# oksuman/FHE-Sorting

Measured on AMD Instinct MI355X. Metric: encrypted sort seconds + ciphertext-mults/sec, N=1024 @ ringDim 2^16, higher is better.
Workload: dtype u64; 1 GPU; DirectSort N=1024, ringDim 2^16, depth 39, scale 2^40, 161 rotation keys, CompositeSign(3, 5, 2), dnum 3, OpenFHE PS split; N=1024, ring_dim=65536, mult_depth=39, scale_bits=40, ps_split=openfhe, special_primes=10, lanes_per_gpu=2, max_stack=32, parallelism=batch-shard x1, collective=none

## Files before the change

### fhe-sorting_amd/csrc/algo/fhesort.cpp

```cpp
#include "fhesort.hpp"

#include <algorithm>
#include <chrono>
#include <cstdio>
#include <cstdlib>
#include <cmath>
#include <fstream>
#include <map>
#include <mutex>
#include <optional>
#include <stdexcept>
#include <tuple>
#include <exception>
#include <thread>

namespace fhe {

namespace {

int ceil_log2(long x) {
    int r = 0;
    while ((1L << r) < x) ++r;
    return r;
}
void trim_zeros(std::vector<double> &a) {
    while (a.size() > 1 && a.back() == 0.0) a.pop_back();
}
size_t ps_chunk() {
    static const size_t v = [] {
        const char *e = std::getenv("FHE_PS_CHUNK");
        const int c = e ? std::atoi(e) : 32;
        return (size_t)std::min(32, std::max(1, c));
    }();
    return v;
}
bool fold_scalars() {
    static const bool v = [] {
        const char *e = std::getenv("FHE_MUL_FOLD_SCALARS");
        return e ? std::atoi(e) != 0 : true;
    }();
    return v;
}

int openfhe_ps_depth(int d) {
    if (d < 5) return ceil_log2(d) + 1;
    static const int band_top[] = {5, 13, 27, 59, 119, 247, 495, 1007, 2031, 2204};
    for (int i = 0; i < 10; ++i)
        if (d <= band_top[i]) return 3 + i;
    const double f = std::floor(std::log2(std::sqrt(d / 2.0)));
    long best = -1;
    int depth = 0;
    for (long k = 1; k <= d; ++k) {
        if (std::fabs(std::floor(std::log2((double)k)) - f) > 1) continue;
// ... 107 lines not shown
                chunk.push_back(i);
        std::vector<int> idx;
        for (size_t c : chunk)
            for (size_t i = 1; i < leaves[c].a.size(); ++i)
                if (leaves[c].a[i] != 0.0) idx.push_back((int)i);
        std::sort(idx.begin(), idx.end());
        idx.erase(std::unique(idx.begin(), idx.end()), idx.end());
        std::vector<const Ciphertext *> xs;
        for (int i : idx) xs.push_back(T.at(i).get());
        std::vector<std::vector<double>> rows;
        for (size_t c : chunk) {
            std::vector<double> row;
            for (int i : idx) row.push_back((size_t)i < leaves[c].a.size() ? leaves[c].a[i] : 0.0);
            rows.push_back(row);
        }
        auto outs = cc.linear_sums_to(xs, rows, target, !raw);
        for (size_t g = 0; g < chunk.size(); ++g) {
            CtPtr r = std::move(outs[g]);
            if (!raw && leaves[chunk[g]].a[0] != 0.0) cc.add_const_inplace(r, leaves[chunk[g]].a[0]);
            ready[chunk[g]] = r;
        }
    }
    CtPtr leaf() {
        const size_t i = next_leaf++;
        const Leaf &L = leaves.at(i);
        if (!has_terms(L.a)) {
            CtPtr r = cc.trivial_const(0.0, L.target, T[1]->slots, T[1]->batch);
            if (L.a[0] != 0.0) cc.add_const_inplace(r, L.a[0]);
            return r;
        }
        if (!ready.count(i)) evaluate_chunk(i);
        CtPtr r = ready.at(i);
        ready.erase(i);
        return r;
// ... 284 lines not shown
        for (size_t c : chunk)
            for (int i = 1; i <= k; ++i)
                if (P->leaves[c].a[i] != 0.0) idx.push_back(i);
        std::sort(idx.begin(), idx.end());
        idx.erase(std::unique(idx.begin(), idx.end()), idx.end());
        const int target = lk + L0.mm - 1 + (L0.raw ? 1 : 0);
        if (idx.empty()) throw std::logic_error("openfhe split: leaf without T terms");
        std::vector<const Ciphertext *> xs;
        for (int i : idx) xs.push_back(T[i].get());
        std::vector<std::vector<double>> rows;
        for (size_t c : chunk) {
            std::vector<double> row;
            for (int i : idx) row.push_back(P->leaves[c].a[i]);
            rows.push_back(row);
        }
        auto outs = cc.linear_sums_to(xs, rows, target, !L0.raw);
        for (size_t g = 0; g < chunk.size(); ++g) {
            CtPtr r = std::move(outs[g]);
            if (!L0.raw && P->leaves[chunk[g]].a[0] != 0.0) cc.add_const_inplace(r, P->leaves[chunk[g]].a[0]);
            ready[chunk[g]] = r;
        }
    }
    CtPtr leaf(int i) {
        if (!ready.count(i)) evaluate_chunk(i);
        CtPtr r = ready.at(i);
        ready.erase(i);
        return r;
    }
    CtPtr node(const OFNode &N) {
        CtPtr cu = N.cu >= 0 ? leaf(N.cu) : nullptr;
        const CtPtr &a = T2[N.mm - 1];
        const double c0 = cu ? 0.0 : N.c0;
        CtPtr qu = N.qn ? node(*N.qn) : leaf(N.qleaf);
        if (N.sn) {
// ... 1791 lines not shown
```

### fhe-sorting_amd/csrc/device/kernels.hip

```cpp
#include <fcntl.h>
#include <signal.h>
#include <sys/syscall.h>
#include <ucontext.h>
#include <unistd.h>

#include <atomic>
#include <cstdlib>
#include <mutex>
#include "kernels.hpp"

#include <cstdlib>
#include <stdexcept>
#include <utility>
#include <type_traits>
#include <string>

namespace fhe {
namespace dev {

namespace {

constexpr int NT = 256;
inline int conv_chunk(int logN, int targets, int zdim) {
    static const int force = [] {
// ... 422 lines not shown
    for (int i = 0; i < A.m; ++i) {
        const ulonglong2 x = ld2(A.x[i] + xo);
        mac128(r0, x.x, w[i]);
        mac128(r1, x.y, w[i]);
    }
    st2(out + off + k, make_ulonglong2(reduce128(r0, md), reduce128(r1, md)));
}
constexpr int MLS_G = 10, MLS_M = 32;
struct MultiLinArgs {
    u64 *out[MLS_G];
    const u64 *x[MLS_M];
    size_t xseg[MLS_M];
    int64_t K[MLS_G * MLS_M];
    uint8_t sh[MLS_G * MLS_M];
    int m, G, accumulate;
};
template <int G>
__global__ __launch_bounds__(NT) void k_linear_sum_multi(MultiLinArgs A, size_t seg, const Mod *mods, int logN) {
    __shared__ Split30 w[G * MLS_M];
    const size_t n = (size_t)1 << logN;
    const int l = blockIdx.y;
    const Mod md = mods[l];
    for (int t = threadIdx.x; t < G * MLS_M; t += NT) w[t] = split30((t % MLS_M) < A.m ? smod(A.K[t], A.sh[t], md) : 0);
    __syncthreads();
    const size_t k = (size_t)blockIdx.x * NT + threadIdx.x;
    if (k >= n) return;
    const size_t ln = (size_t)l * n + k, oo = (size_t)blockIdx.z * seg + ln;
    Acc128 run[G];
#pragma unroll
    for (int g = 0; g < G; ++g) run[g].lo = A.accumulate ? A.out[g][oo] : 0;
    for (int base = 0; base < A.m; base += 16) {
        const int end = min(A.m, base + 16);
        Acc4 s[G];
        u64 xv[16];
#pragma unroll
        for (int u = 0; u < 16; ++u) xv[u] = base + u < end ? A.x[base + u][(size_t)blockIdx.z * A.xseg[base + u] + ln] : 0;
#pragma unroll
        for (int u = 0; u < 16; ++u) {
            if (base + u < end) {
                const Split30 x = split30(xv[u]);
#pragma unroll
                for (int g = 0; g < G; ++g) mac4(s[g], x, w[g * MLS_M + base + u]);
            }
        }
#pragma unroll
// ... 97 lines not shown

__device__ __forceinline__ v4i bytes_hilo(u64 y0, u64 y1) {
    return v4i{(int)(uint32_t)(y0 >> 32), (int)(uint32_t)(y1 >> 32), (int)(uint32_t)y0, (int)(uint32_t)y1};
}
typedef int v16i __attribute__((ext_vector_type(16)));

constexpr int LS_CH_MAX = 4096;
struct LeafArgs {
    u64 *out[LEAF_G];
    const u64 *x[LEAF_M];
    uint32_t xseg[LEAF_M];
    const int64_t *K;
    const uint8_t *sh;
    int m, G, accumulate;
    int six;
};
#ifndef FHE_LF_NC
#define FHE_LF_NC 2
#endif
constexpr int LF_NC = FHE_LF_NC, LF_NT = 256;
#ifndef FHE_LF_WPE
#define FHE_LF_WPE 3
#endif
template <int KS, int NG>
__global__ __launch_bounds__(LF_NT) __attribute__((amdgpu_waves_per_eu(FHE_LF_WPE, 8))) void k_leaf_sums_mfma(LeafArgs A, size_t seg, const Mod *mods, int logN,
                                                          int chunk) {
    __shared__ u64 etab[4 * NG][8 * KS];
    __shared__ u64 corr[4 * NG];
    __shared__ const u64 *xptr[8 * KS];
    __shared__ size_t xoff[8 * KS];
    __shared__ u64 *optr[4 * NG];
// ... 6 lines not shown
        const int t = p / (8 * KS), i = p % (8 * KS);
        const u64 c = (t < A.G && i < A.m) ? smod(A.K[t * A.m + i], A.sh[t * A.m + i], md) : 0;
        etab[t][i] = __builtin_bswap64(balanced_digits(c));
    }
    if (tid < 8 * KS) {
        const int i = tid < A.m ? tid : 0;
        xptr[tid] = A.x[i];
        xoff[tid] = (size_t)blockIdx.z * A.xseg[i] + (size_t)l * n;
    }
    __syncthreads();
    if (tid < 4 * ngr) {
        optr[tid] = tid < A.G ? A.out[tid] : nullptr;
        u64 s = 0;
        if (tid < A.G)
            for (int i = 0; i < A.m; ++i) s = add_mod(s, smod(A.K[tid * A.m + i], A.sh[tid * A.m + i], md), md.q);
        corr[tid] = sums_constant(s, md);
    }
    __syncthreads();
    const int lane = tid & 63, wave = tid >> 6, col = lane & 15, lg = lane >> 4;
    const int ta = (lane & 15) >> 2, rr = lane & 3;
    const uint32_t ab = 3 - rr;
    const u64 w1s = shoup_one(md);
    const size_t oo_l = (size_t)blockIdx.z * seg + (size_t)l * n;
    for (size_t nb = (size_t)blockIdx.x * chunk + wave * 16 * LF_NC; nb < (size_t)(blockIdx.x + 1) * chunk && nb < n;
         nb += LF_NT / 4 * LF_NC) {
        v4i bf[LF_NC][KS];
#pragma unroll
        for (int ks = 0; ks < KS; ++ks) {
            const int i0 = 8 * ks + 2 * lg;
            const gu64 *p0 = to_global(xptr[i0]) + xoff[i0] + nb + col;
            const gu64 *p1 = to_global(xptr[i0 + 1]) + xoff[i0 + 1] + nb + col;
// ... 182 lines not shown
                img[2 * (((grp * 2 + (b >> 2)) * KS + ks) * 64 + lane) + half] = e;
            }
        }
    }
    if (tid < 8 * KS) {
        const int i = tid < A.m ? tid : 0;
        xptr[tid] = A.x[i];
        xoff[tid] = (size_t)blockIdx.z * A.xseg[i] + (size_t)l * n;
    }
    __syncthreads();
    if (tid < 4 * ngr) {
        optr[tid] = tid < A.G ? A.out[tid] : nullptr;
        u64 s = 0;
        for (int i = 0; i < A.m; ++i) s = add_mod(s, psum[tid][i], md.q);
        const u64 b126 = mul_shoup(reduce64(1ull << 62, md), md.r64, md.r64s, md.q);
        corr[tid] = sub_mod(mul_barrett(s, 128, md), b126, md.q);
        cfp[tid] = mul_barrett(s, 128, md);
    }
    __syncthreads();
    const int lane = tid & 63, wave = tid >> 6, col = lane & 15, lg = lane >> 4;
    const u64 w1s = shoup_one(md);
    const double qd = (double)md.q, qid = 1.0 / qd;
    const size_t oo_l = (size_t)blockIdx.z * seg + (size_t)l * n;
    for (size_t nb = (size_t)blockIdx.x * chunk + wave * 16 * LFF_NC; nb < (size_t)(blockIdx.x + 1) * chunk && nb < n;
         nb += LFF_NT / 4 * LFF_NC) {
        v4i bf[LFF_NC][KS];
#pragma unroll
        for (int ks = 0; ks < KS; ++ks) {
            const int i0 = 8 * ks + 2 * lg;
            const gu64 *p0 = to_global(xptr[i0]) + xoff[i0] + nb + col;
            const gu64 *p1 = to_global(xptr[i0 + 1]) + xoff[i0 + 1] + nb + col;
#pragma unroll
// ... 1804 lines not shown
        launch_clocked("k_linear_sum", B, k_linear_sum, ew_grid(logN, limbs, segs), dim3(NT), st, out, A, seg, mods,
                       logN);
        if (m == 0) break;
    }
}
int leaf_fold_enabled() {
    static const int v = [] {
        const char *e = std::getenv("FHE_LEAF_FOLD");
        return e ? std::atoi(e) : 1;
    }();
    return v;
}
bool linear_sums_on_mfma(int logN) { return use_mfma_sums(MF_LIN) && logN >= 8; }
void ew_linear_sum_multi(u64 *const *outs, int G, const u64 *const *xs, const size_t *xseg, const int64_t *K, int m,
                         int limbs, int segs, size_t seg, const Mod *mods, int logN, hipStream_t st,
                         const uint8_t *sh, const int64_t *dK, const uint8_t *dsh) {
    if (limbs <= 0 || segs <= 0 || G <= 0 || m <= 0) return;
    if (G > LEAF_G) throw std::invalid_argument("ew_linear_sum_multi: at most LEAF_G outputs per call");
    const size_t n = (size_t)1 << logN;
    if (linear_sums_on_mfma(logN) && dK && dsh && m <= LEAF_M) {
        {
            LeafArgs A{};
            A.m = m;
            A.G = G;
            A.accumulate = 0;
            for (int g = 0; g < G; ++g) A.out[g] = outs[g];
            A.six = leaf_six_enabled_host();
            for (int i = 0; i < A.m; ++i) {
                A.x[i] = xs[i];
                A.xseg[i] = (uint32_t)xseg[i];
            }
            A.K = dK;
            A.sh = dsh;
            const double B = 8.0 * (A.m + (double)G * (1 + A.accumulate)) * limbs * segs * (double)n;
            size_t ch = std::min<size_t>(LS_CH_MAX, n);
            while (ch > 256 && (n / ch) * (size_t)limbs * (size_t)segs < 2048) ch /= 2;
            const dim3 grid((unsigned)((n + ch - 1) / ch), (unsigned)limbs, (unsigned)segs);
            const int ngc = (G + 3) / 4 <= 1 ? 1 : (G + 3) / 4 <= 2 ? 2 : (G + 3) / 4 <= 4 ? 3 : 4;
            if (leaf_fold_enabled() && n >= 2 * (size_t)LFF_NT) {
                size_t chf = std::min<size_t>(LS_CH_MAX, n);
                while (chf > 2 * (size_t)LFF_NT && (n / chf) * (size_t)limbs * (size_t)segs < 1024) chf /= 2;
                const dim3 gridf((unsigned)((n + chf - 1) / chf), (unsigned)limbs, (unsigned)segs);
                dispatch_int<1, 8>((A.m + 7) / 8, [&](auto ks) {
                    dispatch_int<1, 4>(ngc, [&](auto ng) {
                        constexpr int KS = decltype(ks)::value, NG = 1 << (decltype(ng)::value - 1);
                        launch_clocked(inst_name<KS, NG>("k_leaf_sums_fold"), B, k_leaf_sums_fold<KS, NG>, gridf,
                                       dim3(LFF_NT), st, A, seg, mods, logN, (int)chf);
                    });
// ... 5 lines not shown
                    constexpr int KS = decltype(ks)::value, NG = 1 << (decltype(ng)::value - 1);
                    launch_clocked(inst_name<KS, NG>("k_leaf_sums_mfma"), B, k_leaf_sums_mfma<KS, NG>, grid, dim3(LF_NT),
                                   st, A, seg, mods, logN, (int)ch);
                });
            });
        }
        return;
    }
    for (int g0 = 0; g0 < G; g0 += MLS_G) {
        const int Gp = std::min(MLS_G, G - g0);
        for (int base = 0; base < m; base += MLS_M) {
            MultiLinArgs A{};
            A.m = std::min(MLS_M, m - base);
            A.G = Gp;
            A.accumulate = base > 0;
            for (int g = 0; g < Gp; ++g) A.out[g] = outs[g0 + g];
            for (int i = 0; i < A.m; ++i) {
                A.x[i] = xs[base + i];
                A.xseg[i] = xseg[base + i];
                for (int g = 0; g < Gp; ++g) {
                    A.K[g * MLS_M + i] = K[(size_t)(g0 + g) * m + base + i];
                    A.sh[g * MLS_M + i] = sh ? sh[(size_t)(g0 + g) * m + base + i] : 0;
                }
            }
            const double B = 8.0 * (A.m + (double)Gp * (1 + A.accumulate)) * limbs * segs * (double)n;
            const dim3 grid = pt_grid(logN, limbs, segs);
            switch (Gp) {
#define MLS_CASE(g)                                                                                               \
    case g:                                                                                                       \
        launch_clocked(inst_name<g>("k_linear_sum_multi"), B, k_linear_sum_multi<g>, grid, dim3(NT), st, A, seg, mods, \
// ... 723 lines not shown
```

### fhe-sorting_amd/csrc/device/kernels.hpp

```cpp
#pragma once
#include <string>
#include <utility>
#include <vector>
#include <hip/hip_runtime.h>
#include <hip/hip_ext.h>
#include <cstddef>
#include <cstdint>

#include "modmath.hpp"

namespace fhe {
namespace dev {

struct NttTables {
    const ulonglong2 *fwd2;
    const ulonglong2 *inv2;
    const u64 *ninv, *ninv_s;
    const Mod *mods;
    int logN;
    const double *fwdd = nullptr, *invd = nullptr;
    const double2 *qd = nullptr;
    const uint8_t *fp_host = nullptr;
};
bool ntt_fp_prime(u64 q);
// ... 54 lines not shown
    size_t seg_d = 0;
    const u64 *c1 = nullptr, *c1s = nullptr;
    const u64 *c2 = nullptr, *c2s = nullptr;
    const u64 *src = nullptr;
    size_t seg_src = 0;
    int64_t scalar = 0;
    int scalar_sh = 0;
    bool raw = false;
    int lsegb = 0, segs = 0;
    int zs0 = 0, zn0 = 1 << 30, zs1 = 0;
    __host__ __device__ int limb_of(int z) const { return z < zn0 ? zs0 + z : zs1 + (z - zn0); }
    const u64 *d2 = nullptr;
    size_t seg_d2 = 0;
    const u64 *key = nullptr;
    int nall = 0;
};
void ntt_inverse_from(u64 *dst, const u64 *src, size_t seg_src, int limbs, int segs, size_t seg, const int *pmap,
                      const NttTables &T, hipStream_t st, bool raw = false);
void ntt_forward_rescale(u64 *tmp, int limbs, int segs, const NttFuse &F, const NttTables &T, hipStream_t st);
void ntt_forward_multail(u64 *corr, int limbs, int segs, const NttFuse &F, const NttTables &T, hipStream_t st);
void ntt_forward_multail_own(u64 *corr, int limbs, int segs, const NttFuse &F, const NttTables &T, hipStream_t st);
void ntt_forward_ksfinish(u64 *conv, int limbs, int segs, const NttFuse &F, const NttTables &T, hipStream_t st);
void ntt_row_pass(u64 *data, int limbs, int segs, size_t seg, const int *pmap, const NttTables &T, hipStream_t st,
                  bool forward);
void ntt_forward_mapped(u64 *data, int count, int segs, size_t seg, const int *smap, const int *pmap,
                        const NttTables &T, hipStream_t st);

struct Seg {
    size_t o, a, b;
};
// ... 22 lines not shown
                   const u64 *const *xs, const int64_t *K, const uint8_t *sh, int m, size_t xseg, const Mod *mods,
                   int logN, hipStream_t st, const u64 *a2 = nullptr, size_t sa2 = 0, int64_t aK = 0, int ash = 0,
                   int64_t oK = 0, int osh = 0);
void ew_sum_members(u64 *out, const u64 *in, int members, int limbs, const Mod *mods, int logN, hipStream_t st);
int tensor_cols_per_thread();
void ew_tensor_cols(u64 *d01, u64 *d2, const u64 *a, const u64 *const *cols, int P, int limbs, int members, size_t sa,
                    const Mod *mods, int logN, hipStream_t st);
void ew_sum_member_groups(u64 *out, const u64 *in, int groups, int per_group, int limbs, bool accumulate,
                          const Mod *mods, int logN, hipStream_t st);
void ew_linear_sum(u64 *out, const u64 *const *xs, const int64_t *K, int m, int limbs, int segs, size_t seg,
                   size_t xseg, const Mod *mods, int logN, hipStream_t st, bool accumulate = false,
                   const uint8_t *sh = nullptr);
constexpr int LEAF_G = 32, LEAF_M = 64;
void ew_linear_sum_multi(u64 *const *outs, int G, const u64 *const *xs, const size_t *xseg, const int64_t *K, int m,
                         int limbs, int segs, size_t seg, const Mod *mods, int logN, hipStream_t st,
                         const uint8_t *sh, const int64_t *dK, const uint8_t *dsh);
bool linear_sums_on_mfma(int logN);
void ew_mul_plain_sum(u64 *out, const u64 *const *cts, const u64 *const *pts, int m, int limbs, int members,
                      size_t cmember, size_t cpoly, const Mod *mods, int logN, hipStream_t st);
int plain_sum_tile();
double plain_sum_batches_limb_units(int m, int nb, int tile);
void ew_mul_plain_sum_batches(u64 *out, const u64 *const *cts, const u64 *const *pts, int m, int nb, int limbs,
                              size_t cpoly, const Mod *mods, int logN, hipStream_t st);
int plain_sum_groups_tile();
void ew_mul_plain_sum_groups(u64 *out, const u64 *in, const u64 *const *pts, int m, int groups, int limbs,
                             const Mod *mods, int logN, hipStream_t st);
int sub_add_plain_tile();
void ew_sub_add_plain_stacked(u64 *out, const u64 *a, const u64 *const *bs, const u64 *const *ps, int members,
                              int limbs, const Mod *mods, int logN, hipStream_t st);
int sub_pm_const_tile();
void ew_sub_pm_const_stacked(u64 *out, const u64 *a, const u64 *const *bs, int members, int64_t K, int sh, int limbs,
// ... 106 lines not shown
```

### fhe-sorting_amd/csrc/device/ntt.hip

```cpp
#include <hip/hip_ext.h>

#include <cstdlib>
#include <map>
#include <atomic>
#include <mutex>
#include <stdexcept>
#include <string>
#include <type_traits>
#include <utility>
#include <vector>

#include "kernels.hpp"

namespace fhe {
namespace dev {

namespace {

constexpr int NTB = 256;

template <int Lo, int Hi, typename F>
void dispatch_int(int v, F &&f) {
    if constexpr (Lo > Hi) {
        throw std::invalid_argument("unsupported digit count " + std::to_string(v));
// ... 348 lines not shown
template <bool FWD>
__device__ __forceinline__ int row_final_index(int t, int r) {
    constexpr RowLayout L = row_layout<FWD>(FWD ? 8 : 7);
    return lane_index(L, t) + reg_index(L, r);
}
int &row_shfl_enabled() {
    static int v = [] {
        const char *e = std::getenv("FHE_NTT_ROW_SHFL");
        return e ? std::atoi(e) : 15;
    }();
    return v;
}

enum { NTT_PLAIN = 0, NTT_LIFT = 1, NTT_RESCALE = 2, NTT_MULTAIL = 3, NTT_KSFINISH = 4, NTT_MULTAIL_OWN = 5 };

template <int PB, int EB, bool COLS, int MODE, bool SH, bool FULL, bool TWL = false, bool FP = false>
__device__ __forceinline__ void ntt_fwd_body(u64 *data, size_t seg, const int *pmap, const int *smap, int logN,
                                             const NttTables &Tb, const NttFuse &F) {
    static_assert(!SH || (!COLS && PB == 8 && EB == 4), "shuffle row pass: 16 lanes x 16 coefficients");
    constexpr int E = 1 << EB;
    constexpr int RB = PB - EB;
    constexpr int T = 1 << RB;
    constexpr int NB = nthreads<PB, COLS>() / T;
    constexpr int G = E >> RB;
    constexpr int LEN = 1 << PB;
    constexpr bool SPLIT = COLS && G >= 2;
    constexpr int TPB = SPLIT ? PB - (EB - RB) : PB;
    constexpr bool X32 = lds32<COLS>() && !SPLIT;
    __shared__ u64 tile[SH ? 1 : X32 ? (lds_words<TPB, NB, COLS>() + 1) / 2 : lds_words<TPB, NB, COLS>()];
    uint32_t *const t32 = reinterpret_cast<uint32_t *>(tile);
    constexpr bool CTW = FHE_NTT_COL_TWL && COLS && !SPLIT && PB == 8 && nthreads<PB, COLS>() == 256;
    using TW = TwT<FP>;
    __shared__ TW twc[CTW ? 256 : 1];

    const size_t n = (size_t)1 << logN;
    const int k2 = COLS ? logN - PB : 0;
    const int limb = F.limb_of(blockIdx.z);
    const int p = pmap ? __builtin_amdgcn_readfirstlane(pmap[limb]) : limb;
    int t, tr;
    if (COLS) {
        tr = threadIdx.x % NB;
        t = NB == 64 ? __builtin_amdgcn_readfirstlane(threadIdx.x / NB) : threadIdx.x / NB;
    } else {
        tr = threadIdx.x / T;
        t = threadIdx.x % T;
    }
    const int zseg = SH ? (int)blockIdx.x * (1 << F.lsegb) + (tr & ((1 << F.lsegb) - 1)) : (int)blockIdx.x;
    const size_t tid_global = SH ? (size_t)blockIdx.y * (NB >> F.lsegb) + (tr >> F.lsegb)
                                 : (size_t)blockIdx.y * NB + tr;
    const bool valid = FULL || (tid_global < ((size_t)1 << (logN - PB)) && (!SH || zseg < F.segs));
    u64 *a = data + (size_t)zseg * seg + (smap ? (size_t)__builtin_amdgcn_readfirstlane(smap[limb]) : (size_t)limb) * n;
    const u64 q = Tb.mods[p].q, q2 = 2 * q, q4 = 4 * q, nq = (u64)0 - q;
    const TW *tw;
    if constexpr (FP) tw = Tb.fwdd + (size_t)p * n;
    else tw = Tb.fwd2 + (size_t)p * n;
    Ar A{q4, nq, 0.0, 0.0};
    if constexpr (FP) {
        const double2 qd = Tb.qd[p];
        A.q = qd.x;
        A.qi = qd.y;
    }
    const double fin = FP ? FP_TWO52 + (COLS ? FP_FWD_COL_IN : FP_FWD_COL_OUT) * A.q : 0.0;
    constexpr bool CBUF = FHE_NTT_COL_BUF && COLS && FULL;
    const int S0 = COLS ? 0 : logN - PB;
    if (CTW) twc[threadIdx.x] = tw[threadIdx.x];

    u64 x[E];
    if (MODE == NTT_LIFT) {
        const Mod ml = Tb.mods[F.lastp];
        const u64 ql = ml.q, qh = ql >> 1;
        const u64 kl = F.scalar ? smod64(F.scalar, F.scalar_sh, ml) : 0;
        const u64 *src = F.last + (size_t)zseg * F.seg_last;
        const auto rs = limb_rsrc(src);
        const int vo = (int)((((size_t)t << k2) + tid_global) * 8);
#pragma unroll
        for (int r = 0; r < E; ++r) {
            const int idx = t + T * r;
            u64 c = CBUF ? bload64(rs, vo, (T * r << k2) * 8)
                         : valid ? src[(size_t)idx * ((size_t)1 << k2) + tid_global] : 0;
            if (F.scalar) c = mul_barrett(c, kl, ml);
            x[r] = c > qh ? q - (ql - c) : c;
        }
    } else if constexpr (CBUF) {
// ... 394 lines not shown
            v = scale ? mul_shoup(x[r], ni, nis, q) : COLS ? (x[r] >= q2 ? x[r] - q2 : x[r]) : x[r];
        }
        if constexpr (CBUF)
            bstore64(rso, vso, (T * r << k2) * 8, v);
        else if (valid)
            a[off] = v;
    }
}

#ifndef FHE_NTT_COL_WPE
#define FHE_NTT_COL_WPE 1
#endif
template <int PB, int EB, bool COLS, int MODE, bool FULL, bool FP>
__global__ __launch_bounds__((nthreads<PB, COLS>())) __attribute__((amdgpu_waves_per_eu(COLS ? FHE_NTT_COL_WPE : 1, 8))) void k_ntt_fwd(
    u64 *data, size_t seg, const int *pmap, const int *smap, int logN, NttTables Tb, NttFuse F) {
    ntt_fwd_body<PB, EB, COLS, MODE, false, FULL, false, FP>(data, seg, pmap, smap, logN, Tb, F);
}
template <int PB, int EB, bool COLS, bool FULL, bool FP>
__global__ __launch_bounds__((nthreads<PB, COLS>())) __attribute__((amdgpu_waves_per_eu(COLS ? FHE_NTT_COL_WPE : 1, 8))) void k_ntt_inv(
    u64 *data, size_t seg, const int *pmap, const int *smap, int logN, NttTables Tb, NttFuse F) {
    ntt_inv_body<PB, EB, COLS, false, FULL, false, FP>(data, seg, pmap, smap, logN, Tb, F);
}
#ifndef FHE_NTT_ROW_WPE
#define FHE_NTT_ROW_WPE 1
#endif
#ifndef FHE_NTT_FP_ROW_WPE
#define FHE_NTT_FP_ROW_WPE 1
#endif
#ifndef FHE_NTT_FP_RESCALE_WPE
#define FHE_NTT_FP_RESCALE_WPE FHE_NTT_FP_ROW_WPE
#endif
template <int MODE, bool FULL, bool TWL, bool FP>
__global__ __launch_bounds__(NTB) __attribute__((amdgpu_waves_per_eu(FP ? (MODE == NTT_RESCALE ? FHE_NTT_FP_RESCALE_WPE : FHE_NTT_FP_ROW_WPE) : TWL ? FHE_NTT_ROW_WPE : 1, 8))) void k_ntt_fwd_row(
    u64 *data, size_t seg, const int *pmap, const int *smap, int logN, NttTables Tb, NttFuse F) {
    ntt_fwd_body<8, 4, false, MODE, true, FULL, TWL, FP>(data, seg, pmap, smap, logN, Tb, F);
}
template <bool FULL, bool TWL, bool FP>
__global__ __launch_bounds__(NTB) __attribute__((amdgpu_waves_per_eu(TWL ? FHE_NTT_ROW_WPE : 1, 8))) void k_ntt_inv_row(
    u64 *data, size_t seg, const int *pmap, const int *smap, int logN, NttTables Tb, NttFuse F) {
    ntt_inv_body<8, 4, false, true, FULL, TWL, FP>(data, seg, pmap, smap, logN, Tb, F);
}
#ifndef FHE_ROW_KS_WPE
#define FHE_ROW_KS_WPE 2
#endif
#ifndef FHE_ROW_KS_WPE1
#define FHE_ROW_KS_WPE1 4
#endif
template <int D, bool FP, bool FULL>
__global__ __launch_bounds__(NTB) __attribute__((amdgpu_waves_per_eu(D == 1 ? FHE_ROW_KS_WPE1 : FHE_ROW_KS_WPE, 8))) void k_ntt_row_ks(u64 *acc, const u64 *ext, const u64 *dntt, const u64 *key,
                                                    int ell, int W, int nall, int alpha, int members,
// ... 154 lines not shown
int &ntt_full_mask() {
    static int v = [] {
        const char *e = std::getenv("FHE_NTT_FULL");
        return e ? std::atoi(e) : 53 | 128;
    }();
    return v;
}
template <bool COLS, bool FWD, int MODE>
constexpr int full_bit() {
    return FWD ? (COLS ? (MODE == NTT_LIFT ? 2 : 1)
                       : MODE == NTT_RESCALE ? 8 : (MODE == NTT_MULTAIL || MODE == NTT_MULTAIL_OWN) ? 16
                       : MODE == NTT_KSFINISH ? 128 : 4)
               : (COLS ? 32 : 64);
}

template <int PB, int EB, bool COLS, bool FWD, int MODE, bool FP>
void launch_pass_one(u64 *data, int limbs, int segs, size_t seg, const int *pmap, const int *smap, const NttTables &T,
                     const NttFuse &F, hipStream_t st) {
    constexpr int NTHR = nthreads<PB, COLS>();
    constexpr int NB = NTHR >> (PB - EB);
    constexpr bool CAN_SH = !COLS && PB == 8 && EB == 4;
    const int mode = row_shfl_enabled();
    const int fwd_bit = (MODE == NTT_MULTAIL || MODE == NTT_MULTAIL_OWN) ? 4 : MODE == NTT_RESCALE ? 8
                        : MODE == NTT_KSFINISH ? 16 : 0;
    const bool sh = CAN_SH && (mode & (FWD ? 2 | fwd_bit : 1)) != 0;
    const int count = 1 << (T.logN - PB);
    dim3 grid((unsigned)segs, (unsigned)((count + NB - 1) / NB), (unsigned)limbs);
    const bool want_full = (ntt_full_mask() & full_bit<COLS, FWD, MODE>()) != 0;
    bool full = want_full && count % NB == 0;
    NttFuse Fs = F;
    if (sh) {
        Fs.lsegb = 0;
        while (Fs.lsegb < 4 && (2 << Fs.lsegb) <= segs) ++Fs.lsegb;
        Fs.segs = segs;
        const int rows_pb = NB >> Fs.lsegb;
        grid = dim3((unsigned)((segs + (1 << Fs.lsegb) - 1) >> Fs.lsegb), (unsigned)((count + rows_pb - 1) / rows_pb),
                    (unsigned)limbs);
        full = want_full && count % rows_pb == 0 && segs % (1 << Fs.lsegb) == 0;
    }
    LaunchClock *clk = launch_clock();
    hipEvent_t e0 = nullptr, e1 = nullptr;
    const int slot = clk ? clk->events(e0, e1) : -1;
    note_launch(FWD ? (COLS ? "k_ntt_fwd(col)" : "k_ntt_fwd(row)") : (COLS ? "k_ntt_inv(col)" : "k_ntt_inv(row)"), grid,
                dim3(NTHR));
    const int rows_blk = 16 >> Fs.lsegb;
    const bool twl = sh && rows_blk <= row_twl_rows() && row_twl_enabled() != 0;
    const unsigned lds_dyn = twl ? (unsigned)(rows_blk * 256 * (FP ? sizeof(double) : sizeof(TwT<false>))) : 0u;
#define FHE_NTT_LAUNCH(K, FF) \
    hipExtLaunchKernelGGL((K), grid, dim3(NTHR), lds_dyn, st, e0, e1, 0, data, seg, pmap, smap, T.logN, T, FF)
    if (FWD && sh) {
        if (full && twl) FHE_NTT_LAUNCH((k_ntt_fwd_row<MODE, true, true, FP>), Fs);
        else if (full) FHE_NTT_LAUNCH((k_ntt_fwd_row<MODE, true, false, FP>), Fs);
        else if (twl) FHE_NTT_LAUNCH((k_ntt_fwd_row<MODE, false, true, FP>), Fs);
        else FHE_NTT_LAUNCH((k_ntt_fwd_row<MODE, false, false, FP>), Fs);
    } else if (FWD) {
        if (full) FHE_NTT_LAUNCH((k_ntt_fwd<PB, EB, COLS, MODE, true, FP>), F);
        else FHE_NTT_LAUNCH((k_ntt_fwd<PB, EB, COLS, MODE, false, FP>), F);
    } else if (sh) {
        if (full && twl) FHE_NTT_LAUNCH((k_ntt_inv_row<true, true, FP>), Fs);
        else if (full) FHE_NTT_LAUNCH((k_ntt_inv_row<true, false, FP>), Fs);
        else if (twl) FHE_NTT_LAUNCH((k_ntt_inv_row<false, true, FP>), Fs);
        else FHE_NTT_LAUNCH((k_ntt_inv_row<false, false, FP>), Fs);
    } else {
        if (full) FHE_NTT_LAUNCH((k_ntt_inv<PB, EB, COLS, true, FP>), F);
        else FHE_NTT_LAUNCH((k_ntt_inv<PB, EB, COLS, false, FP>), F);
    }
#undef FHE_NTT_LAUNCH
    if (clk) {
        const std::string fps = FP ? "true>" : "false>";
        const std::string pe = std::to_string(PB) + ", " + std::to_string(EB) + (COLS ? ", true" : ", false");
        const std::string fl = (full ? "true, " : "false, ") + fps;
        const std::string fl2 = (full ? "true, " : "false, ") + std::string(twl ? "true, " : "false, ") + fps;
        const std::string base = FWD && sh ? "k_ntt_fwd_row<" + std::to_string(MODE) + ", " + fl2
                                 : FWD     ? "k_ntt_fwd<" + pe + ", " + std::to_string(MODE) + ", " + fl
                                 : sh      ? "k_ntt_inv_row<" + fl2
                                           : "k_ntt_inv<" + pe + ", " + fl;
        static std::map<std::string, std::string> names;
        static std::mutex mu;
        const char *ph = launch_phase();
        const std::string key = ph ? base + "@" + ph : base;
        std::lock_guard<std::mutex> lk(mu);
        auto it = names.find(key);
        if (it == names.end()) it = names.emplace(key, key).first;
        const double extra = MODE == NTT_RESCALE ? 1.0 : MODE == NTT_MULTAIL ? 2.0
                             : MODE == NTT_KSFINISH || MODE == NTT_MULTAIL_OWN ? 1.5 : 0.0;
        const double once = MODE == NTT_MULTAIL_OWN ? 2.0 : 0.0;
        clk->record(slot, it->second.c_str(),
                    ((2.0 + extra) * segs + once) * 8.0 * (double)limbs * ((size_t)1 << T.logN));
    }
}

int &ntt_fp_enabled() {
    static int v = [] {
        const char *e = std::getenv("FHE_NTT_FP");
        return e ? std::atoi(e) : 1;
    }();
    return v;
}
struct MapRegistry {
    std::mutex mu;
    std::map<const int *, std::vector<int>> maps;
    std::atomic<unsigned long> gen{0};
};
// ... 339 lines not shown
```

### fhe-sorting_amd/csrc/engine/engine.hip

```cpp
#include <hip/hip_runtime.h>

#include <algorithm>
#include <atomic>
#include <chrono>
#include <cmath>
#include <cstring>
#include <map>
#include <mutex>
#include <set>
#include <stdexcept>
#include <functional>
#include <thread>

#include "../device/kernels.hpp"
#include "engine.hpp"

#define HIP_OK(x)                                                                                     \
    do {                                                                                              \
        hipError_t _e = (x);                                                                          \
        if (_e != hipSuccess)                                                                         \
            throw std::runtime_error(std::string("HIP error ") + hipGetErrorString(_e) + " at " +    \
                                     __FILE__ + ":" + std::to_string(__LINE__));                      \
    } while (0)

// ... 2163 lines not shown
        } else {
            auto sm = I.alloc((size_t)segs * ell * nn * 8);
            u64 *s = static_cast<u64 *>(sm->p);
            dev::ew_linear_sum(s, p.data(), k.data(), (int)p.size(), (int)ell, segs, ell * nn, kv.first * nn, MODS,
                               LOGN, ST, false, sh.data());
            dev::ew_add(t, t, s, (int)ell, segs, seg3(ell * nn, ell * nn, ell * nn), MODS, LOGN, ST);
        }
    }
    ctr.rescale += B;
    auto r = new_ct(target, xs[0]->slots, I.P.delta[target], ell - 1, B);
    I.rescale(t, ell, ell * nn, segs, r->data);
    return r;
}

std::vector<CtPtr> Engine::linear_sums_to(const std::vector<const Ciphertext *> &xs,
                                          const std::vector<std::vector<double>> &c, int target, bool rescale) {
    auto &I = *impl;
    if (target > I.P.L) throw std::runtime_error("linear_sums_to: no levels left");
    if (xs.empty()) throw std::invalid_argument("linear_sums_to: no inputs");
    const int B = xs[0]->batch, segs = 2 * B;
    const size_t nn = n(), ell = I.P.limbs_at(target - 1), m = xs.size();
    const u64 qd = I.P.primes[I.P.L - target + 1];
    count_bytes((2.0 * ell * m + 2.0 * ell) * c.size(), B);
    std::vector<const u64 *> xp(m);
    std::vector<size_t> xseg(m);
    for (size_t i = 0; i < m; ++i) {
        if (xs[i]->level > target - 1) throw std::invalid_argument("linear_sums_to: input level too high");
        if (xs[i]->batch != B) throw std::invalid_argument("linear_sums_to: batch size mismatch");
        xp[i] = xs[i]->data;
        xseg[i] = xs[i]->limbs * nn;
    }
    std::vector<CtPtr> outs;
    const size_t passes = (c.size() + dev::LEAF_G - 1) / dev::LEAF_G, per = (c.size() + passes - 1) / passes;
    const bool mfma = dev::linear_sums_on_mfma(LOGN) && m <= (size_t)dev::LEAF_M;
    for (size_t g0 = 0; g0 < c.size(); g0 += per) {
        const int G = (int)std::min<size_t>(per, c.size() - g0);
        std::vector<int64_t> K((size_t)G * m);
        std::vector<uint8_t> sh((size_t)G * m);
        for (int g = 0; g < G; ++g) {
            if (c[g0 + g].size() != m) throw std::invalid_argument("linear_sums_to: coefficient row size");
            for (size_t i = 0; i < m; ++i) {
                const host::SConst k = host::const_to_target(c[g0 + g][i], I.P.delta[target], qd, xs[i]->scale);
                K[(size_t)g * m + i] = k.k;
                sh[(size_t)g * m + i] = (uint8_t)k.sh;
            }
        }
        auto tm = I.alloc((size_t)G * segs * ell * nn * 8);
        u64 *t = static_cast<u64 *>(tm->p);
        std::vector<u64 *> op(G);
        for (int g = 0; g < G; ++g) op[g] = t + (size_t)g * segs * ell * nn;
        std::pair<const int64_t *, const uint8_t *> dk{nullptr, nullptr};
        if (mfma) dk = I.const_table(K, sh);
        dev::ew_linear_sum_multi(op.data(), G, xp.data(), xseg.data(), K.data(), (int)m, (int)ell, segs, ell * nn,
                                 MODS, LOGN, ST, sh.data(), dk.first, dk.second);
        if (!rescale) {
            for (int g = 0; g < G; ++g) {
                auto r = std::make_shared<Ciphertext>();
                r->mem = tm;
                r->data = op[g];
                r->level = target - 1;
                r->slots = xs[0]->slots;
                r->scale = I.P.delta[target] * (double)qd;
                r->limbs = ell;
                r->batch = B;
                outs.push_back(r);
            }
            ctr.constmult += (u64)G * m * B;
            continue;
        }
// ... 532 lines not shown
```

### fhe-sorting_amd/csrc/engine/engine.hpp

```cpp
#pragma once
#include <array>
#include <complex>
#include <cstddef>
#include <cstdint>
#include <memory>
#include <stdexcept>
#include <string>
#include <vector>

#include "../host/hostmath.hpp"

namespace fhe {

using u64 = uint64_t;
using i64 = int64_t;
using PublicSeed = std::array<uint8_t, 32>;

struct DevMem;

struct Ciphertext {
    std::shared_ptr<DevMem> mem;
    u64 *data = nullptr;
    int level = 0;
    int slots = 0;
// ... 140 lines not shown
    CtPtr rotate_members(const Ciphertext &a, const std::vector<long> &ks);
    CtPtr rotate_sum_hoisted(const Ciphertext &x, const std::vector<long> &ks);
    struct LtGiant {
        long shift = 0;
        std::vector<int> baby;
        std::vector<const Plaintext *> pts;
    };
    CtPtr linear_transform_ext(const Ciphertext &x, const std::vector<long> &baby, const std::vector<LtGiant> &giants);
    std::vector<CtPtr> apply_galois_hoisted(const Ciphertext &a, const std::vector<u64> &gs);
    CtPtr conjugate(const Ciphertext &a);
    CtPtr mod_raise(const Ciphertext &a);
    CtPtr rescale(const Ciphertext &a);
    CtPtr drop_to(const Ciphertext &a, int level);
    CtPtr linear_sum_to(const std::vector<const Ciphertext *> &xs, const std::vector<double> &c, int target);
    std::vector<CtPtr> linear_sums_to(const std::vector<const Ciphertext *> &xs,
                                      const std::vector<std::vector<double>> &c, int target, bool rescale = true);
    CtPtr trivial_const(double c, int level, int slots, int batch = 1);
    CtPtr zero_like(int level, int slots, int batch = 1);
    CtPtr stack(const std::vector<const Ciphertext *> &xs);
    CtPtr member(const Ciphertext &a, int m);
    CtPtr sub_stacked(const Ciphertext &a, const std::vector<const Ciphertext *> &bs);
    CtPtr sub_plain_stacked(const Ciphertext &a, const std::vector<const Plaintext *> &ps);
    CtPtr sub_add_plain_stacked(const Ciphertext &a, const std::vector<const Ciphertext *> &bs,
                                const std::vector<const Plaintext *> &ps);
    CtPtr sub_pm_const_stacked(const Ciphertext &a, const std::vector<const Ciphertext *> &bs, double c);
    CtPtr sum_members(const Ciphertext &a);
    void sum_member_groups(const Ciphertext &a, int groups, CtPtr &acc);
    void reduce_after_allreduce(Ciphertext &ct);

    void ntt_host(u64 *data, int prime_index, int limbs, bool inverse);
    void modup_host(const u64 *d, size_t ell, u64 *ext);
// ... 44 lines not shown
```

Measured before the change: 10990 ciphertext-mults/s.

## Fold leaf constants into linear-sum kernels and loop lifted NTT over limbs

```diff
diff --git a/fhe-sorting_amd/csrc/algo/fhesort.cpp b/fhe-sorting_amd/csrc/algo/fhesort.cpp
--- a/fhe-sorting_amd/csrc/algo/fhesort.cpp
+++ b/fhe-sorting_amd/csrc/algo/fhesort.cpp
@@ -37,6 +37,13 @@
 bool fold_scalars() {
     static const bool v = [] {
         const char *e = std::getenv("FHE_MUL_FOLD_SCALARS");
+        return e ? std::atoi(e) != 0 : true;
+    }();
+    return v;
+}
+bool leaf_const_fold() {
+    static const bool v = [] {
+        const char *e = std::getenv("FHE_LEAF_CONST_FOLD");
         return e ? std::atoi(e) != 0 : true;
     }();
     return v;
@@ -174,10 +181,13 @@
             for (int i : idx) row.push_back((size_t)i < leaves[c].a.size() ? leaves[c].a[i] : 0.0);
             rows.push_back(row);
         }
-        auto outs = cc.linear_sums_to(xs, rows, target, !raw);
+        const bool fold = !raw && leaf_const_fold();
+        std::vector<double> a0;
+        for (size_t c : chunk) a0.push_back(leaves[c].a[0]);
+        auto outs = cc.linear_sums_to(xs, rows, target, !raw, fold ? &a0 : nullptr);
         for (size_t g = 0; g < chunk.size(); ++g) {
             CtPtr r = std::move(outs[g]);
-            if (!raw && leaves[chunk[g]].a[0] != 0.0) cc.add_const_inplace(r, leaves[chunk[g]].a[0]);
+            if (!raw && !fold && a0[g] != 0.0) cc.add_const_inplace(r, a0[g]);
             ready[chunk[g]] = r;
         }
     }
@@ -492,10 +502,13 @@
             for (int i : idx) row.push_back(P->leaves[c].a[i]);
             rows.push_back(row);
         }
-        auto outs = cc.linear_sums_to(xs, rows, target, !L0.raw);
+        const bool fold = !L0.raw && leaf_const_fold();
+        std::vector<double> a0;
+        for (size_t c : chunk) a0.push_back(P->leaves[c].a[0]);
+        auto outs = cc.linear_sums_to(xs, rows, target, !L0.raw, fold ? &a0 : nullptr);
         for (size_t g = 0; g < chunk.size(); ++g) {
             CtPtr r = std::move(outs[g]);
-            if (!L0.raw && P->leaves[chunk[g]].a[0] != 0.0) cc.add_const_inplace(r, P->leaves[chunk[g]].a[0]);
+            if (!L0.raw && !fold && a0[g] != 0.0) cc.add_const_inplace(r, a0[g]);
             ready[chunk[g]] = r;
         }
     }
diff --git a/fhe-sorting_amd/csrc/device/kernels.hip b/fhe-sorting_amd/csrc/device/kernels.hip
--- a/fhe-sorting_amd/csrc/device/kernels.hip
+++ b/fhe-sorting_amd/csrc/device/kernels.hip
@@ -460,21 +460,32 @@
     int64_t K[MLS_G * MLS_M];
     uint8_t sh[MLS_G * MLS_M];
     int m, G, accumulate;
+    int64_t Kc[MLS_G];
+    uint8_t shc[MLS_G];
+    int cfold;
+    u64 qlast;
 };
+__device__ __forceinline__ u64 const_times_qlast(int64_t K, int sh, u64 qlast, const Mod &md) {
+    return mul_barrett(smod(K, sh, md), reduce64(qlast, md), md);
+}
 template <int G>
 __global__ __launch_bounds__(NT) void k_linear_sum_multi(MultiLinArgs A, size_t seg, const Mod *mods, int logN) {
     __shared__ Split30 w[G * MLS_M];
+    __shared__ u64 cadd[G];
     const size_t n = (size_t)1 << logN;
     const int l = blockIdx.y;
     const Mod md = mods[l];
     for (int t = threadIdx.x; t < G * MLS_M; t += NT) w[t] = split30((t % MLS_M) < A.m ? smod(A.K[t], A.sh[t], md) : 0);
+    if (threadIdx.x < G)
+        cadd[threadIdx.x] = (A.cfold && !(blockIdx.z & 1) && l < A.cfold)
+                                ? const_times_qlast(A.Kc[threadIdx.x], A.shc[threadIdx.x], A.qlast, md) : 0;
     __syncthreads();
     const size_t k = (size_t)blockIdx.x * NT + threadIdx.x;
     if (k >= n) return;
     const size_t ln = (size_t)l * n + k, oo = (size_t)blockIdx.z * seg + ln;
     Acc128 run[G];
 #pragma unroll
-    for (int g = 0; g < G; ++g) run[g].lo = A.accumulate ? A.out[g][oo] : 0;
+    for (int g = 0; g < G; ++g) run[g].lo = (A.accumulate ? A.out[g][oo] : 0) + cadd[g];
     for (int base = 0; base < A.m; base += 16) {
         const int end = min(A.m, base + 16);
         Acc4 s[G];
@@ -602,7 +613,13 @@
     const uint8_t *sh;
     int m, G, accumulate;
     int six;
+    int cfold;
+    u64 qlast;
 };
+__device__ __forceinline__ u64 leaf_const(const LeafArgs &A, int t, int l, const Mod &md) {
+    if (!A.cfold || t >= A.G || (blockIdx.z & 1) || l >= A.cfold) return 0;
+    return const_times_qlast(A.K[A.G * A.m + t], A.sh[A.G * A.m + t], A.qlast, md);
+}
 #ifndef FHE_LF_NC
 #define FHE_LF_NC 2
 #endif
@@ -639,7 +656,7 @@
         u64 s = 0;
         if (tid < A.G)
             for (int i = 0; i < A.m; ++i) s = add_mod(s, smod(A.K[tid * A.m + i], A.sh[tid * A.m + i], md), md.q);
-        corr[tid] = sums_constant(s, md);
+        corr[tid] = add_mod(sums_constant(s, md), leaf_const(A, tid, l, md), md.q);
     }
     __syncthreads();
     const int lane = tid & 63, wave = tid >> 6, col = lane & 15, lg = lane >> 4;
@@ -852,8 +869,9 @@
         u64 s = 0;
         for (int i = 0; i < A.m; ++i) s = add_mod(s, psum[tid][i], md.q);
         const u64 b126 = mul_shoup(reduce64(1ull << 62, md), md.r64, md.r64s, md.q);
-        corr[tid] = sub_mod(mul_barrett(s, 128, md), b126, md.q);
-        cfp[tid] = mul_barrett(s, 128, md);
+        const u64 ca = leaf_const(A, tid, l, md);
+        corr[tid] = add_mod(sub_mod(mul_barrett(s, 128, md), b126, md.q), ca, md.q);
+        cfp[tid] = add_mod(mul_barrett(s, 128, md), ca, md.q);
     }
     __syncthreads();
     const int lane = tid & 63, wave = tid >> 6, col = lane & 15, lg = lane >> 4;
@@ -2688,7 +2706,7 @@
 bool linear_sums_on_mfma(int logN) { return use_mfma_sums(MF_LIN) && logN >= 8; }
 void ew_linear_sum_multi(u64 *const *outs, int G, const u64 *const *xs, const size_t *xseg, const int64_t *K, int m,
                          int limbs, int segs, size_t seg, const Mod *mods, int logN, hipStream_t st,
-                         const uint8_t *sh, const int64_t *dK, const uint8_t *dsh) {
+                         const uint8_t *sh, const int64_t *dK, const uint8_t *dsh, int cfold, u64 qlast) {
     if (limbs <= 0 || segs <= 0 || G <= 0 || m <= 0) return;
     if (G > LEAF_G) throw std::invalid_argument("ew_linear_sum_multi: at most LEAF_G outputs per call");
     const size_t n = (size_t)1 << logN;
@@ -2706,6 +2724,8 @@
             }
             A.K = dK;
             A.sh = dsh;
+            A.cfold = cfold;
+            A.qlast = qlast;
             const double B = 8.0 * (A.m + (double)G * (1 + A.accumulate)) * limbs * segs * (double)n;
             size_t ch = std::min<size_t>(LS_CH_MAX, n);
             while (ch > 256 && (n / ch) * (size_t)limbs * (size_t)segs < 2048) ch /= 2;
@@ -2741,6 +2761,12 @@
             A.m = std::min(MLS_M, m - base);
             A.G = Gp;
             A.accumulate = base > 0;
+            A.cfold = base == 0 ? cfold : 0;
+            A.qlast = qlast;
+            for (int g = 0; g < Gp && cfold; ++g) {
+                A.Kc[g] = K[(size_t)G * m + g0 + g];
+                A.shc[g] = sh ? sh[(size_t)G * m + g0 + g] : 0;
+            }
             for (int g = 0; g < Gp; ++g) A.out[g] = outs[g0 + g];
             for (int i = 0; i < A.m; ++i) {
                 A.x[i] = xs[base + i];
diff --git a/fhe-sorting_amd/csrc/device/kernels.hpp b/fhe-sorting_amd/csrc/device/kernels.hpp
--- a/fhe-sorting_amd/csrc/device/kernels.hpp
+++ b/fhe-sorting_amd/csrc/device/kernels.hpp
@@ -92,6 +92,7 @@
     size_t seg_d2 = 0;
     const u64 *key = nullptr;
     int nall = 0;
+    int zchunk = 1, zcount = 0;
 };
 void ntt_inverse_from(u64 *dst, const u64 *src, size_t seg_src, int limbs, int segs, size_t seg, const int *pmap,
                       const NttTables &T, hipStream_t st, bool raw = false);
@@ -144,7 +145,7 @@
 constexpr int LEAF_G = 32, LEAF_M = 64;
 void ew_linear_sum_multi(u64 *const *outs, int G, const u64 *const *xs, const size_t *xseg, const int64_t *K, int m,
                          int limbs, int segs, size_t seg, const Mod *mods, int logN, hipStream_t st,
-                         const uint8_t *sh, const int64_t *dK, const uint8_t *dsh);
+                         const uint8_t *sh, const int64_t *dK, const uint8_t *dsh, int cfold = 0, u64 qlast = 0);
 bool linear_sums_on_mfma(int logN);
 void ew_mul_plain_sum(u64 *out, const u64 *const *cts, const u64 *const *pts, int m, int limbs, int members,
                       size_t cmember, size_t cpoly, const Mod *mods, int logN, hipStream_t st);
diff --git a/fhe-sorting_amd/csrc/device/ntt.hip b/fhe-sorting_amd/csrc/device/ntt.hip
--- a/fhe-sorting_amd/csrc/device/ntt.hip
+++ b/fhe-sorting_amd/csrc/device/ntt.hip
@@ -386,9 +386,12 @@
 
 enum { NTT_PLAIN = 0, NTT_LIFT = 1, NTT_RESCALE = 2, NTT_MULTAIL = 3, NTT_KSFINISH = 4, NTT_MULTAIL_OWN = 5 };
 
-template <int PB, int EB, bool COLS, int MODE, bool SH, bool FULL, bool TWL = false, bool FP = false>
+template <int PB, int EB, bool COLS, int MODE, bool SH, bool FULL, bool TWL = false, bool FP = false,
+          bool LOOPED = false>
 __device__ __forceinline__ void ntt_fwd_body(u64 *data, size_t seg, const int *pmap, const int *smap, int logN,
-                                             const NttTables &Tb, const NttFuse &F) {
+                                             const NttTables &Tb, const NttFuse &F, const int zi,
+                                             const u64 *raw = nullptr) {
+    static_assert(!LOOPED || (COLS && MODE == NTT_LIFT), "looped body: the lifted column pass");
     static_assert(!SH || (!COLS && PB == 8 && EB == 4), "shuffle row pass: 16 lanes x 16 coefficients");
     constexpr int E = 1 << EB;
     constexpr int RB = PB - EB;
@@ -407,7 +410,7 @@
 
     const size_t n = (size_t)1 << logN;
     const int k2 = COLS ? logN - PB : 0;
-    const int limb = F.limb_of(blockIdx.z);
+    const int limb = F.limb_of(zi);
     const int p = pmap ? __builtin_amdgcn_readfirstlane(pmap[limb]) : limb;
     int t, tr;
     if (COLS) {
@@ -438,7 +441,11 @@
     if (CTW) twc[threadIdx.x] = tw[threadIdx.x];
 
     u64 x[E];
-    if (MODE == NTT_LIFT) {
+    if constexpr (LOOPED) {
+        const u64 ql = Tb.mods[F.lastp].q, qh = ql >> 1;
+#pragma unroll
+        for (int r = 0; r < E; ++r) x[r] = raw[r] > qh ? q - (ql - raw[r]) : raw[r];
+    } else if (MODE == NTT_LIFT) {
         const Mod ml = Tb.mods[F.lastp];
         const u64 ql = ml.q, qh = ql >> 1;
         const u64 kl = F.scalar ? smod64(F.scalar, F.scalar_sh, ml) : 0;
@@ -863,7 +870,30 @@
 template <int PB, int EB, bool COLS, int MODE, bool FULL, bool FP>
 __global__ __launch_bounds__((nthreads<PB, COLS>())) __attribute__((amdgpu_waves_per_eu(COLS ? FHE_NTT_COL_WPE : 1, 8))) void k_ntt_fwd(
     u64 *data, size_t seg, const int *pmap, const int *smap, int logN, NttTables Tb, NttFuse F) {
-    ntt_fwd_body<PB, EB, COLS, MODE, false, FULL, false, FP>(data, seg, pmap, smap, logN, Tb, F);
+    ntt_fwd_body<PB, EB, COLS, MODE, false, FULL, false, FP>(data, seg, pmap, smap, logN, Tb, F, blockIdx.z);
+}
+template <int PB, int EB, bool FP>
+__global__ __launch_bounds__((nthreads<PB, true>())) __attribute__((amdgpu_waves_per_eu(FHE_NTT_COL_WPE, 8))) void k_ntt_lift_loop(
+    u64 *data, size_t seg, const int *pmap, const int *smap, int logN, NttTables Tb, NttFuse F) {
+    constexpr int E = 1 << EB, T = 1 << (PB - EB), NB = nthreads<PB, true>() / T;
+    const int k2 = logN - PB;
+    const int tr = threadIdx.x % NB, t = threadIdx.x / NB;
+    const size_t col = (size_t)blockIdx.y * NB + tr;
+    const u64 *src = F.last + (size_t)blockIdx.x * F.seg_last;
+    const Mod ml = Tb.mods[F.lastp];
+    const u64 kl = F.scalar ? smod64(F.scalar, F.scalar_sh, ml) : 0;
+    u64 raw[E];
+#pragma unroll
+    for (int r = 0; r < E; ++r) {
+        u64 c = src[((size_t)(t + T * r) << k2) + col];
+        if (F.scalar) c = mul_barrett(c, kl, ml);
+        raw[r] = c;
+    }
+    const int z0 = (int)blockIdx.z * F.zchunk, z1 = min(z0 + F.zchunk, F.zcount);
+    for (int z = z0; z < z1; ++z) {
+        if (z != z0) __syncthreads();
+        ntt_fwd_body<PB, EB, true, NTT_LIFT, false, true, false, FP, true>(data, seg, pmap, smap, logN, Tb, F, z, raw);
+    }
 }
 template <int PB, int EB, bool COLS, bool FULL, bool FP>
 __global__ __launch_bounds__((nthreads<PB, COLS>())) __attribute__((amdgpu_waves_per_eu(COLS ? FHE_NTT_COL_WPE : 1, 8))) void k_ntt_inv(
@@ -882,7 +912,7 @@
 template <int MODE, bool FULL, bool TWL, bool FP>
 __global__ __launch_bounds__(NTB) __attribute__((amdgpu_waves_per_eu(FP ? (MODE == NTT_RESCALE ? FHE_NTT_FP_RESCALE_WPE : FHE_NTT_FP_ROW_WPE) : TWL ? FHE_NTT_ROW_WPE : 1, 8))) void k_ntt_fwd_row(
     u64 *data, size_t seg, const int *pmap, const int *smap, int logN, NttTables Tb, NttFuse F) {
-    ntt_fwd_body<8, 4, false, MODE, true, FULL, TWL, FP>(data, seg, pmap, smap, logN, Tb, F);
+    ntt_fwd_body<8, 4, false, MODE, true, FULL, TWL, FP>(data, seg, pmap, smap, logN, Tb, F, blockIdx.z);
 }
 template <bool FULL, bool TWL, bool FP>
 __global__ __launch_bounds__(NTB) __attribute__((amdgpu_waves_per_eu(TWL ? FHE_NTT_ROW_WPE : 1, 8))) void k_ntt_inv_row(
@@ -1067,6 +1097,21 @@
                : (COLS ? 32 : 64);
 }
 
+int &lift_loop_enabled() {
+    static int v = [] {
+        const char *e = std::getenv("FHE_RESCALE_LIFT_LOOP");
+        return e ? std::atoi(e) : 1;
+    }();
+    return v;
+}
+int &lift_loop_min_blocks() {
+    static int v = [] {
+        const char *e = std::getenv("FHE_RESCALE_LIFT_MIN_BLOCKS");
+        return e ? std::max(1, std::atoi(e)) : 2048;
+    }();
+    return v;
+}
+
 template <int PB, int EB, bool COLS, bool FWD, int MODE, bool FP>
 void launch_pass_one(u64 *data, int limbs, int segs, size_t seg, const int *pmap, const int *smap, const NttTables &T,
                      const NttFuse &F, hipStream_t st) {
@@ -1091,17 +1136,29 @@
                     (unsigned)limbs);
         full = want_full && count % rows_pb == 0 && segs % (1 << Fs.lsegb) == 0;
     }
+    constexpr bool CAN_LOOP = COLS && FWD && MODE == NTT_LIFT && PB >= 6 && PB <= 8;
+    bool loop = false;
+    if (CAN_LOOP && limbs > 1 && count % NB == 0 && lift_loop_enabled() != 0) {
+        const long tiles = (long)grid.x * grid.y;
+        const long nz = std::min<long>(limbs, (lift_loop_min_blocks() + tiles - 1) / tiles);
+        Fs.zchunk = (int)((limbs + nz - 1) / nz);
+        Fs.zcount = limbs;
+        loop = Fs.zchunk > 1;
+        if (loop) grid.z = (unsigned)((limbs + Fs.zchunk - 1) / Fs.zchunk);
+    }
     LaunchClock *clk = launch_clock();
     hipEvent_t e0 = nullptr, e1 = nullptr;
     const int slot = clk ? clk->events(e0, e1) : -1;
-    note_launch(FWD ? (COLS ? "k_ntt_fwd(col)" : "k_ntt_fwd(row)") : (COLS ? "k_ntt_inv(col)" : "k_ntt_inv(row)"), grid,
+    note_launch(loop ? "k_ntt_lift_loop(col)" : FWD ? (COLS ? "k_ntt_fwd(col)" : "k_ntt_fwd(row)") : (COLS ? "k_ntt_inv(col)" : "k_ntt_inv(row)"), grid,
                 dim3(NTHR));
     const int rows_blk = 16 >> Fs.lsegb;
     const bool twl = sh && rows_blk <= row_twl_rows() && row_twl_enabled() != 0;
     const unsigned lds_dyn = twl ? (unsigned)(rows_blk * 256 * (FP ? sizeof(double) : sizeof(TwT<false>))) : 0u;
 #define FHE_NTT_LAUNCH(K, FF) \
     hipExtLaunchKernelGGL((K), grid, dim3(NTHR), lds_dyn, st, e0, e1, 0, data, seg, pmap, smap, T.logN, T, FF)
-    if (FWD && sh) {
+    if (loop) {
+        if constexpr (CAN_LOOP) FHE_NTT_LAUNCH((k_ntt_lift_loop<PB, EB, FP>), Fs);
+    } else if (FWD && sh) {
         if (full && twl) FHE_NTT_LAUNCH((k_ntt_fwd_row<MODE, true, true, FP>), Fs);
         else if (full) FHE_NTT_LAUNCH((k_ntt_fwd_row<MODE, true, false, FP>), Fs);
         else if (twl) FHE_NTT_LAUNCH((k_ntt_fwd_row<MODE, false, true, FP>), Fs);
@@ -1124,7 +1181,8 @@
         const std::string pe = std::to_string(PB) + ", " + std::to_string(EB) + (COLS ? ", true" : ", false");
         const std::string fl = (full ? "true, " : "false, ") + fps;
         const std::string fl2 = (full ? "true, " : "false, ") + std::string(twl ? "true, " : "false, ") + fps;
-        const std::string base = FWD && sh ? "k_ntt_fwd_row<" + std::to_string(MODE) + ", " + fl2
+        const std::string base = loop      ? "k_ntt_lift_loop<" + std::to_string(PB) + ", " + std::to_string(EB) + ", " + fps
+                                 : FWD && sh ? "k_ntt_fwd_row<" + std::to_string(MODE) + ", " + fl2
                                  : FWD     ? "k_ntt_fwd<" + pe + ", " + std::to_string(MODE) + ", " + fl
                                  : sh      ? "k_ntt_inv_row<" + fl2
                                            : "k_ntt_inv<" + pe + ", " + fl;
@@ -1138,8 +1196,9 @@
         const double extra = MODE == NTT_RESCALE ? 1.0 : MODE == NTT_MULTAIL ? 2.0
                              : MODE == NTT_KSFINISH || MODE == NTT_MULTAIL_OWN ? 1.5 : 0.0;
         const double once = MODE == NTT_MULTAIL_OWN ? 2.0 : 0.0;
-        clk->record(slot, it->second.c_str(),
-                    ((2.0 + extra) * segs + once) * 8.0 * (double)limbs * ((size_t)1 << T.logN));
+        const double bytes = loop ? (double)(limbs + 1) * segs * 8.0 * ((size_t)1 << T.logN)
+                                  : ((2.0 + extra) * segs + once) * 8.0 * (double)limbs * ((size_t)1 << T.logN);
+        clk->record(slot, it->second.c_str(), bytes);
     }
 }
 
diff --git a/fhe-sorting_amd/csrc/engine/engine.hip b/fhe-sorting_amd/csrc/engine/engine.hip
--- a/fhe-sorting_amd/csrc/engine/engine.hip
+++ b/fhe-sorting_amd/csrc/engine/engine.hip
@@ -2201,10 +2201,13 @@
 }
 
 std::vector<CtPtr> Engine::linear_sums_to(const std::vector<const Ciphertext *> &xs,
-                                          const std::vector<std::vector<double>> &c, int target, bool rescale) {
+                                          const std::vector<std::vector<double>> &c, int target, bool rescale,
+                                          const std::vector<double> *consts) {
     auto &I = *impl;
     if (target > I.P.L) throw std::runtime_error("linear_sums_to: no levels left");
     if (xs.empty()) throw std::invalid_argument("linear_sums_to: no inputs");
+    if (consts && !rescale) throw std::invalid_argument("linear_sums_to: constants go with rescaled sums only");
+    if (consts && consts->size() != c.size()) throw std::invalid_argument("linear_sums_to: one constant per output");
     const int B = xs[0]->batch, segs = 2 * B;
     const size_t nn = n(), ell = I.P.limbs_at(target - 1), m = xs.size();
     const u64 qd = I.P.primes[I.P.L - target + 1];
@@ -2222,8 +2225,15 @@
     const bool mfma = dev::linear_sums_on_mfma(LOGN) && m <= (size_t)dev::LEAF_M;
     for (size_t g0 = 0; g0 < c.size(); g0 += per) {
         const int G = (int)std::min<size_t>(per, c.size() - g0);
-        std::vector<int64_t> K((size_t)G * m);
-        std::vector<uint8_t> sh((size_t)G * m);
+        std::vector<int64_t> K((size_t)G * m + (consts ? G : 0));
+        std::vector<uint8_t> sh((size_t)G * m + (consts ? G : 0));
+        for (int g = 0; g < G && consts; ++g) {
+            const double cg = (*consts)[g0 + g];
+            const host::SConst k = cg != 0.0 ? host::const_at_scale(cg, I.P.delta[target]) : host::SConst{};
+            K[(size_t)G * m + g] = k.k;
+            sh[(size_t)G * m + g] = (uint8_t)k.sh;
+            if (cg != 0.0) count_bytes(4.0 * (ell - 1), B);
+        }
         for (int g = 0; g < G; ++g) {
             if (c[g0 + g].size() != m) throw std::invalid_argument("linear_sums_to: coefficient row size");
             for (size_t i = 0; i < m; ++i) {
@@ -2239,7 +2249,7 @@
         std::pair<const int64_t *, const uint8_t *> dk{nullptr, nullptr};
         if (mfma) dk = I.const_table(K, sh);
         dev::ew_linear_sum_multi(op.data(), G, xp.data(), xseg.data(), K.data(), (int)m, (int)ell, segs, ell * nn,
-                                 MODS, LOGN, ST, sh.data(), dk.first, dk.second);
+                                 MODS, LOGN, ST, sh.data(), dk.first, dk.second, consts ? (int)ell - 1 : 0, qd);
         if (!rescale) {
             for (int g = 0; g < G; ++g) {
                 auto r = std::make_shared<Ciphertext>();
diff --git a/fhe-sorting_amd/csrc/engine/engine.hpp b/fhe-sorting_amd/csrc/engine/engine.hpp
--- a/fhe-sorting_amd/csrc/engine/engine.hpp
+++ b/fhe-sorting_amd/csrc/engine/engine.hpp
@@ -178,7 +178,8 @@
     CtPtr drop_to(const Ciphertext &a, int level);
     CtPtr linear_sum_to(const std::vector<const Ciphertext *> &xs, const std::vector<double> &c, int target);
     std::vector<CtPtr> linear_sums_to(const std::vector<const Ciphertext *> &xs,
-                                      const std::vector<std::vector<double>> &c, int target, bool rescale = true);
+                                      const std::vector<std::vector<double>> &c, int target, bool rescale = true,
+                                      const std::vector<double> *consts = nullptr);
     CtPtr trivial_const(double c, int level, int slots, int batch = 1);
     CtPtr zero_like(int level, int slots, int batch = 1);
     CtPtr stack(const std::vector<const Ciphertext *> &xs);
```

New measurement: 11280 ciphertext-mults/s (median of 6 runs). 1.03x the previous value.
